# theAdamColton/spiht

Hardware: AMD Instinct MI355X
Metric: Mpixels/sec encode+decode at fixed bpp; bitstream-exact vs Rust ref (higher is better)
Workload: dtype f64 DWT / int32 bit-plane coding; 1 GPU; cfg2 image (1920x1080 RGB, bior2.2 reflect level 7, q=50, 0.5 bpp) x 256 per GPU (cfg4 shard), encode+decode, HBM-resident; images_per_gpu=256, distinct_images_per_gpu=256, seeds=1000 + global image index, streams=1, images_per_launch=256, decoder_waves=8, max_bits=1036800

## Files before the change

### include/spiht_hip.h

```cpp
#ifndef SPIHT_HIP_H
#define SPIHT_HIP_H

#include <stdint.h>

#ifdef __cplusplus
extern "C" {
#endif

enum {
    SPIHT_OK = 0,
    SPIHT_ERR_LL = 1,
    SPIHT_ERR_EMPTY = 2,
    SPIHT_ERR_SHAPE = 3,
    SPIHT_ERR_CAPACITY = 4,
    SPIHT_ERR_HIP = 5,
    SPIHT_ERR_ARG = 6,
    SPIHT_ERR_MAGNITUDE = 7,
    SPIHT_ERR_INTERNAL = 8,
    SPIHT_ERR_TOO_LARGE = 9,
    SPIHT_ERR_NOMEM = 10
};

enum { SPIHT_MODE_REFLECT = 0, SPIHT_MODE_SYMMETRIC = 1, SPIHT_MODE_PERIODIC = 2, SPIHT_MODE_ZERO = 3,
       SPIHT_MODE_CONSTANT = 4,
// ... 423 lines not shown
                          int64_t W, double *d_out);
int spiht_encode_image_batch_flt(spiht_ctx *ctx, int kind, const void *d_img, const int64_t *strides, int64_t B, int64_t c,
                                 int64_t H, int64_t W, int wavelet, int mode, int level, double q_scale,
                                 const double *channel_mults, uint64_t max_bits, uint8_t *d_out, uint64_t slot_stride,
                                 uint64_t *d_nbits, uint8_t *d_max_n, int32_t *d_coeffs);
int spiht_encode_image_host_flt(spiht_ctx *ctx, int kind, const void *img, const int64_t *strides, int64_t c, int64_t H, int64_t W,
                                int wavelet, int mode, int level, double q_scale, const double *channel_mults,
                                uint64_t max_bits, uint8_t *out, uint64_t out_cap, uint64_t *out_nbits, uint8_t *max_n);
int spiht_dwt_pyramid_batch_flt(spiht_ctx *ctx, int kind, const void *d_img, const int64_t *strides, int64_t B, int64_t c, int64_t H,
                                int64_t W, int wavelet, int mode, int level, double q_scale, const double *channel_mults,
                                int32_t *d_coeffs, uint8_t *d_dmsb, uint8_t *d_lmsb, uint32_t *d_maxabs);
int spiht_sse_tiles_flt(spiht_ctx *ctx, int kind, const void *d_tiles, const double *d_dec, int64_t G, int64_t N, int64_t c,
                        int64_t H, int64_t W, int64_t th, int64_t tw, int64_t rh, int64_t rw, double *d_out);
int spiht_sse_tiles_w_flt(spiht_ctx *ctx, int kind, const void *d_tiles, const double *d_dec, int64_t G, int64_t N, int64_t c,
                          int64_t H, int64_t W, int64_t th, int64_t tw, int64_t rh, int64_t rw, double *d_out, const uint8_t *d_w,
                          uint64_t w_stride);
int spiht_tile_cut_f32s(spiht_ctx *ctx, const float *d_img, const int64_t *strides, int64_t N, int64_t c, int64_t H, int64_t W,
                        int64_t th, int64_t tw, float *d_tiles);
int spiht_tile_cut_overlap_f32s(spiht_ctx *ctx, const float *d_img, const int64_t *strides, int64_t N, int64_t c, int64_t H,
                                int64_t W, int64_t th, int64_t tw, int64_t m, float *d_tiles);

int spiht_dwt_addr32(int64_t in_h, int64_t in_w, int64_t out_h, int64_t out_w, int64_t enc_h, int64_t enc_w, int px_es,
                     int64_t px_sh, int64_t px_sw);

enum { SPIHT_ERR_BUSY = 11,
       SPIHT_ERR_TIMEOUT = 12,
       SPIHT_ERR_IDLE = 13 };
enum { SPIHT_HS_ENCODE = 0, SPIHT_HS_DECODE = 1 };
enum { SPIHT_HS_F64 = 0, SPIHT_HS_U8 = 1, SPIHT_HS_U16 = 2,
       SPIHT_HS_FLT32 = 3, SPIHT_HS_FLT16 = 4, SPIHT_HS_BF16 = 5  };
#define SPIHT_HS_DESTROY_MS 10000
typedef struct spiht_hstream spiht_hstream;
typedef struct spiht_hstream_result {
    int64_t n;
    uint64_t nbytes;
    const uint8_t *bytes;
    const uint32_t *lens;
    const uint8_t *max_n;
    void *pictures;
    uint64_t step;
} spiht_hstream_result;
int spiht_hstream_create(spiht_ctx *ctx, int direction, int elem, int64_t B, int depth, int64_t c, int64_t H, int64_t W,
                         int wavelet, int mode, int level, double q_scale, const double *channel_mults, uint64_t max_bits,
                         const int64_t *strides, spiht_hstream **out);
int spiht_hstream_destroy(spiht_hstream *s);
int spiht_hstream_info(spiht_hstream *s, uint64_t *slot_bytes, uint64_t *pic_bytes, int64_t *rec_H, int64_t *rec_W);
// ... 28 lines not shown
```

### spiht_amd/_lib.py

```python
import ctypes as C
import os
import threading

_HERE = os.path.dirname(os.path.abspath(__file__))
LIB_PATH = os.environ.get("SPIHT_HIP_LIB") or os.path.join(_HERE, "libspiht_hip.so")

OK, ERR_LL, ERR_EMPTY, ERR_SHAPE, ERR_CAPACITY, ERR_HIP, ERR_ARG, ERR_MAGNITUDE, ERR_INTERNAL, ERR_TOO_LARGE, \
    ERR_NOMEM = range(11)
ERR_BUSY, ERR_TIMEOUT, ERR_IDLE = 11, 12, 13

MODES = {"reflect": 0, "symmetric": 1, "periodic": 2, "zero": 3, "constant": 4}


class SpihtHipError(RuntimeError):
    """A HIP runtime failure or an internal guard of libspiht_hip."""


class PanicException(BaseException):
    """Counterpart of pyo3_runtime.PanicException, which the reference raises when the Rust core panics
    (assert!(ll_h > 1), encoder_decoder.rs:160-161; out-of-bounds index; unwrap on an empty array).
    Like PyO3's, it derives from BaseException."""


_lib = None
# ... 23 lines not shown
    "spiht_dwt_pyramid_batch_u8", "spiht_dequant_idwt_flags_batch_u8", "spiht_idwt_level1_flags_batch_u8", "spiht_pipeline_submit_u8",
    "spiht_check_view_u8", "spiht_decode_with_metadata_batch_i32",
    "spiht_encode_image_batch_u16", "spiht_decode_image_batch_u16", "spiht_encode_image_host_u16", "spiht_decode_image_host_u16",
    "spiht_dwt_pyramid_batch_u16", "spiht_dequant_idwt_flags_batch_u16", "spiht_idwt_level1_flags_batch_u16", "spiht_pipeline_submit_u16",
    "spiht_check_view_u16",
    "spiht_reduced_shape",
    "spiht_dequant_idwt_reduced_batch_f64", "spiht_dequant_idwt_reduced_batch_u8", "spiht_dequant_idwt_reduced_batch_u16",
    "spiht_decode_image_reduced_batch_f64", "spiht_decode_image_reduced_batch_u8", "spiht_decode_image_reduced_batch_u16",
    "spiht_decode_image_reduced_host_f64", "spiht_decode_image_reduced_host_u8", "spiht_decode_image_reduced_host_u16",
    "spiht_sqerr_i32", "spiht_sse_f64", "spiht_sse_u8", "spiht_sse_u16",
    "spiht_tile_grid", "spiht_tile_cut_u8", "spiht_tile_cut_u16", "spiht_tile_cut_f32", "spiht_tile_cut_f64",
    "spiht_tile_paste_u8", "spiht_tile_paste_u16", "spiht_tile_paste_f32", "spiht_tile_paste_f64",
    "spiht_tile_pack", "spiht_tile_unpack",
    "spiht_tile_reduced_grid", "spiht_tile_mosaic_u8", "spiht_tile_mosaic_u16", "spiht_tile_mosaic_f64",
    "spiht_tile_prefix_slots", "spiht_sse_tiles_f64", "spiht_sse_tiles_u8", "spiht_sse_tiles_u16", "spiht_tile_allocate",
    "spiht_layer_pack", "spiht_layer_unpack",
    "spiht_sse_tiles_w_f64", "spiht_sse_tiles_w_u8", "spiht_sse_tiles_w_u16",
    "spiht_tile_allocate_target",
    "spiht_tile_cut_overlap_u8", "spiht_tile_cut_overlap_u16", "spiht_tile_cut_overlap_f32", "spiht_tile_cut_overlap_f64",
    "spiht_tile_blend_u8", "spiht_tile_blend_u16", "spiht_tile_blend_f64",
    "spiht_check_view_flt", "spiht_convert_batch_flt", "spiht_decode_image_batch_flt", "spiht_decode_image_host_flt",
    "spiht_dequant_idwt_flags_batch_flt", "spiht_dequant_idwt_reduced_batch_flt", "spiht_decode_image_reduced_batch_flt",
    "spiht_decode_image_reduced_host_flt", "spiht_tile_blend_flt", "spiht_tile_paste_f32s", "spiht_tile_mosaic_f32",
    "spiht_dwt_addr32",
    "spiht_widen_batch_flt", "spiht_encode_image_batch_flt", "spiht_encode_image_host_flt", "spiht_dwt_pyramid_batch_flt",
    "spiht_sse_tiles_flt", "spiht_sse_tiles_w_flt", "spiht_tile_cut_f32s", "spiht_tile_cut_overlap_f32s",
    "spiht_hstream_create", "spiht_hstream_destroy", "spiht_hstream_info", "spiht_hstream_input", "spiht_hstream_decode_input",
    "spiht_hstream_submit", "spiht_hstream_next", "spiht_hstream_pending",
    "spiht_tile_cut_set", "spiht_tile_paste_set",
]


class HStreamResult(C.Structure):
    _fields_ = [("n", C.c_int64), ("nbytes", C.c_uint64), ("bytes", C.c_void_p), ("lens", C.c_void_p), ("max_n", C.c_void_p),
                ("pictures", C.c_void_p), ("step", C.c_uint64)]


class TileSetPic(C.Structure):
    _fields_ = [("d_img", C.c_void_p), ("sc", C.c_int64), ("sh", C.c_int64), ("sw", C.c_int64), ("H", C.c_int64), ("W", C.c_int64)]


class TileSetItem(C.Structure):
    _fields_ = [("d_out", C.c_void_p), ("sc", C.c_int64), ("sh", C.c_int64), ("sw", C.c_int64), ("H", C.c_int64), ("W", C.c_int64),
                ("i0", C.c_int64), ("i1", C.c_int64), ("j0", C.c_int64), ("j1", C.c_int64),
                ("y0", C.c_int64), ("x0", C.c_int64), ("wh", C.c_int64), ("ww", C.c_int64)]


# ... 365 lines not shown
```

### spiht_amd/csrc/api_dwt.cpp

```cpp
#include "api_internal.h"
#include "wavelets.h"

static int dwt_max_level(int64_t len, int F) {
    if (F <= 1 || len < F - 1) return 0;
    int64_t q = len / (F - 1);
    int l = 0;
    while (q > 1) { q >>= 1; l++; }
    return l;
}

int img_geometry(int64_t H, int64_t W, int F_real, int level, ImgGeom *g, int mode) {
    if (H < 1 || W < 1) return SPIHT_ERR_ARG;
    int L = level;
    if (L < 0) L = std::min(dwt_max_level(H, F_real), dwt_max_level(W, F_real));
    if (L > SPIHT_MAX_LEVELS) return SPIHT_ERR_ARG;
    g->per = mode == SPIHT_MODE_PERIODIZATION;
    g->l0 = 0;
    const int F = g->per ? 2 : F_real;
    g->L = L;
    g->hs[0] = H;
    g->ws[0] = W;
    for (int l = 1; l <= L; l++) {
        g->hs[l] = (g->hs[l - 1] + F - 1) / 2;
        g->ws[l] = (g->ws[l - 1] + F - 1) / 2;
// ... 380 lines not shown
        CHK(ensure(ctx, ctx->a1, maxa * planes * 8));
    }
    const double *a_in = d_a_in;
    int64_t ah = ig.ll_h, aw = ig.ll_w;
    if (l_hi < ig.L) { ah = 2 * ig.hs[l_hi + 1] - Fg + 2; aw = 2 * ig.ws[l_hi + 1] - Fg + 2; }
    for (int l = l_hi; l >= l_lo; l--) {
        IdwtKArgs a;
        memset(&a, 0, sizeof(a));
        a.c = c;
        a.F = F;
        a.band_h = (int32_t)ig.hs[l]; a.band_w = (int32_t)ig.ws[l];
        a.out_h = (int32_t)(2 * ig.hs[l] - F + 2); a.out_w = (int32_t)(2 * ig.ws[l] - F + 2);
        a.a_h = (int32_t)ah; a.a_w = (int32_t)aw;
        if (!((ah == ig.hs[l] || ah == ig.hs[l] + 1) && (aw == ig.ws[l] || aw == ig.ws[l] + 1))) return SPIHT_ERR_ARG;
        if (ig.per) { a.out_h = (int32_t)(2 * ig.hs[l]); a.out_w = (int32_t)(2 * ig.ws[l]); }
        a.off_h = (int32_t)ig.offh[l]; a.off_w = (int32_t)ig.offw[l];
        a.enc_h = (int32_t)ig.enc_h; a.enc_w = (int32_t)ig.enc_w;
        a.first = (l == ig.L) ? 1 : 0;
        a.a_in = a_in;
        a.rec = d_rec;
        a.out = (l == l_lo) ? d_out : (double *)((l & 1) ? ctx->a1.p : ctx->a0.p);
        a.mults = d_mults;
        a.q = q;
        if (color && l == 1) { a.color = 1; a.col = ctx->col_inv; }
        if (l == 1 && !a.first && !a.color) a.flags = d_flags;
        memcpy(a.lo, wv.rec_lo, sizeof(double) * std::min(F, SPIHT_MAX_TAPS));
        memcpy(a.hi, wv.rec_hi, sizeof(double) * std::min(F, SPIHT_MAX_TAPS));
        const bool conv8 = strided && l == 1 && (ig.per || F > SPIHT_MAX_TAPS);
        if (conv8) {
            CHK(ensure(ctx, ctx->pix, (size_t)planes * a.out_h * a.out_w * 8));
            a.out = (double *)ctx->pix.p;
        }
        if (ig.per || F > SPIHT_MAX_TAPS) {
            const double *d_filt;
            CHK(upload_filters(ctx, wavelet, &d_filt));
            StageTimer t(ctx, l + ig.l0 == 1 ? ST_IDWT_L1 : ST_IDWT_REST);
            a.color = 0;
            const size_t per_plane = (size_t)2 * a.band_h * a.out_w * 8;
            int pc = (int)std::max<size_t>(1, ((size_t)1 << 30) / per_plane);
            pc = std::max(c, pc / c * c);
            CHK(ensure(ctx, ctx->exttmp, per_plane * (size_t)std::min(pc, planes)));
            for (int p0 = 0; p0 < planes; p0 += pc) {
                const int np = std::min(pc, planes - p0);
                IdwtKArgs b = a;
                if (b.a_in) b.a_in = a.a_in + (size_t)p0 * a.a_h * a.a_w;
                b.rec = a.rec + (size_t)p0 * a.enc_h * a.enc_w;
// ... 47 lines not shown
```

### spiht_amd/csrc/common.h

```cpp
#pragma once
#include <hip/hip_runtime.h>
#include <stdint.h>

#define SPIHT_MAX_LEVELS 32
#define SPIHT_MAX_TAPS 20

struct FastDiv {
    uint32_t m, sh, d, pad;
};

static inline FastDiv fastdiv_make(uint32_t d) {
    FastDiv f;
    f.d = d;
    f.pad = 0;
    if (d < 2) { f.m = 0; f.sh = 0; return f; }
    uint32_t l = 0;
    while ((1ull << l) < d) l++;
    uint64_t m = ((1ull << 32) * ((1ull << l) - d)) / d + 1;
    f.m = (uint32_t)m;
    f.sh = l - 1;
    return f;
}

#ifdef __HIPCC__
// ... 233 lines not shown
    int32_t lds_per_cu;
    uint32_t started;
};
#define TILECTR_WORDS (9 * 32)
#define TILECTR_STARTED (8 * 32)
struct TileBase { uint32_t v[8]; };

struct IdwtKArgs {
    int32_t c;
    int32_t F;
    int32_t band_h, band_w;
    int32_t out_h, out_w;
    int32_t a_h, a_w;
    int32_t off_h, off_w, enc_h, enc_w;
    int32_t first;
    int32_t planes;
    const double *a_in;
    const int32_t *rec;
    const uint32_t *flags;
    double *out;
    const double *mults;
    double q;
    double lo[SPIHT_MAX_TAPS], hi[SPIHT_MAX_TAPS];
    int32_t color, pad2;
    Color3 col;
    PxView px;
};

struct LlPicArgs {
    const int32_t *rec;
    int32_t enc_h, enc_w, ll_h, ll_w;
    int32_t c, color;
    const double *mults;
    double q;
    double *out;
    PxView px;
    Color3 col;
};

extern "C" {
int spiht_launch_absmax(const int32_t *d_x, int B, uint32_t n, uint32_t *d_maxabs, hipStream_t st);
int spiht_launch_pyramid(const Geom *g, int B, const int32_t *d_x, uint8_t *d_dmsb, uint8_t *d_lmsb, hipStream_t st);
int spiht_launch_encode(const EncArgs *a, hipStream_t st);
int spiht_launch_encode_wide(const EncArgs *a, const WideArgs *w, int groups, hipStream_t st);
int spiht_wide_groups_per_cu(void);
int spiht_launch_decode(const DecArgs *a, hipStream_t st);
int spiht_launch_decode_w8(const DecArgs *a, hipStream_t st);
int spiht_launch_unscatter(const DecArgs *a, hipStream_t st);
int spiht_meta_sort_temp_bytes(uint64_t rows, size_t *bytes);
int spiht_launch_metadata(const MetaArgs *a, uint32_t *keys_in, uint32_t *vals_in, uint32_t *keys_out, uint32_t *vals_out,
// ... 29 lines not shown
```

### spiht_amd/csrc/dwt_inv.hip

```cpp
#include "dwt_device.h"


template <int F, uint32_t LOM, uint32_t HIM, int PX = PX_F64>
__global__ __launch_bounds__(DW_BLOCK) void k_idwt_level(IdwtKArgs a) {
    constexpr int HF = F / 2;
    constexpr int KH = IW_TH / 2 + HF - 1;
    constexpr int KW = IW_TW / 2 + HF - 1;
    constexpr int KHH = IW_TH / 4 + HF - 1;
    __shared__ double s_b[4][KH][KW + 1];
    uint32_t tbx, tby, tbz;
    xcd_tile((a.out_w + IW_TW - 1) / IW_TW, (a.out_h + IW_TH - 1) / IW_TH, a.planes, tbx, tby, tbz);
    const int plane = (int)tbz;
    const int k = plane % a.c;
    const int m0 = (int)tby * IW_TH, n0 = (int)tbx * IW_TW;
    const int kh0 = m0 / 2, kw0 = n0 / 2;
    const bool has_m = a.mults != nullptr;
    const double mk = has_m ? a.mults[k] : 1.0;
    const bool zero_ok = (!has_m || mk > 0.0) && a.q > 0.0;
    const int32_t *__restrict__ rec = a.rec + (size_t)plane * a.enc_h * a.enc_w;
    const double *__restrict__ ain = a.first ? nullptr : a.a_in + (size_t)plane * a.a_h * a.a_w;
    const int tid = threadIdx.x;
    const bool occupied = a.flags == nullptr ||
        a.flags[((size_t)plane * ((a.out_h + IW_TH - 1) / IW_TH) + tby) * ((a.out_w + IW_TW - 1) / IW_TW) + tbx] != 0u;

// ... 65 lines not shown
                double sa = 0.0, sd = 0.0;
#pragma unroll
                for (int j = 0; j < HF; j++) {
                    const int s = HF - 1 - j;
                    const bool lnz = (LOM >> (mp + F - 2 - 2 * s)) & 1u, hnz = (HIM >> (mp + F - 2 - 2 * s)) & 1u;
                    if (lnz) sa += wl[s] * a.lo[mp + F - 2 - 2 * s];
                    if (hnz) sd += wh[s] * a.hi[mp + F - 2 - 2 * s];
                }
                const double sacc = (0.0 + sa) + sd;
                if (PX) {
                    if (m + mp < a.px.h && n < a.px.w) PX_STORE(PX, out8, (int64_t)(m + mp) * a.px.sh + (int64_t)n * a.px.sw, sacc, a.px.kind);
                } else {
                    if (m + mp < a.out_h && n < a.out_w) out[(size_t)(m + mp) * a.out_w + n] = sacc;
                }
            }
        }
    }
}

#ifndef IWP_WG
#define IWP_WG 4
#endif

template <int F, uint32_t LOM, uint32_t HIM, bool FIRST, bool FLAGS = false, int PX = PX_F64>
__global__ __launch_bounds__(DW_BLOCK) void k_idwt_level_pf(IdwtKArgs a, uint32_t gx, uint32_t gy, uint32_t *ctr,
                                                                      TileBase cb) {
    static_assert(!(FIRST && FLAGS), "the flags are those of level 1 of a transform with two levels or more");
    constexpr int HF = F / 2;
    constexpr int KH = IW_TH / 2 + HF - 1, KW = IW_TW / 2 + HF - 1, KHH = IW_TH / 4 + HF - 1;
    constexpr int NE = (KH * KW + DW_BLOCK - 1) / DW_BLOCK;
    __shared__ double s_b[4][KH][KW + 1];
    const int tid = threadIdx.x;
    const uint32_t nt = gx * gy * (uint32_t)a.planes;
    const uint32_t x = blockIdx.x & 7u, q = nt >> 3, r8 = nt & 7u;
    const uint32_t base = x * q + (x < r8 ? x : r8), cnt = q + (x < r8 ? 1u : 0u);
    __shared__ uint32_t s_next[2];
    uint32_t *const myctr = ctr + 32u * x;
    const uint32_t cbase = cb.v[x];
    if (tid == 0) atomicAdd(ctr + TILECTR_STARTED, 1u);
    uint32_t k, kn;
    if (tid == 0) {
        s_next[0] = atomicAdd(myctr, 1u) - cbase;
        s_next[1] = atomicAdd(myctr, 1u) - cbase;
    }
    __syncthreads();
    k = __builtin_amdgcn_readfirstlane(s_next[0]);
    kn = __builtin_amdgcn_readfirstlane(s_next[1]);
    __syncthreads();

    struct Stage {
        int32_t rad[NE], rda[NE], rdd[NE], raa[NE];
        double vaa[NE];
        double mk;
    };
    auto request = [&](Stage &g, uint32_t T, uint32_t occ) {
        const uint32_t bx = T % gx, t2 = T / gx, by = t2 % gy, plane = t2 / gy;
        const int kh0 = (int)(by * IW_TH) / 2, kw0 = (int)(bx * IW_TW) / 2;
        const int32_t *__restrict__ rec = a.rec + (size_t)plane * a.enc_h * a.enc_w;
        const double *__restrict__ ain = FIRST ? nullptr : a.a_in + (size_t)plane * a.a_h * a.a_w;
        const __amdgpu_buffer_rsrc_t rrsrc = plane_rsrc(rec, (uint32_t)a.enc_h * (uint32_t)a.enc_w * 4u);
#pragma unroll
        for (int e = 0; e < NE; e++) {
            const int p = min(tid + e * DW_BLOCK, KH * KW - 1);
            const int rr = p / KW, cidx = p - rr * KW;
            const int bi = min(kh0 + rr, a.band_h - 1), bj = min(kw0 + cidx, a.band_w - 1);
            if (FLAGS) {
                const uint32_t o_ad = ((uint32_t)bi * (uint32_t)a.enc_w + (uint32_t)(a.off_w + bj)) * 4u;
                const uint32_t o_da = ((uint32_t)(a.off_h + bi) * (uint32_t)a.enc_w + (uint32_t)bj) * 4u;
                g.rad[e] = __builtin_amdgcn_raw_buffer_load_b32(rrsrc, occ ? o_ad : BUF_OOB, 0, 0);
                g.rda[e] = __builtin_amdgcn_raw_buffer_load_b32(rrsrc, occ ? o_da : BUF_OOB, 0, 0);
                g.rdd[e] = __builtin_amdgcn_raw_buffer_load_b32(rrsrc, occ ? o_da + (uint32_t)a.off_w * 4u : BUF_OOB, 0, 0);
            } else {
                g.rad[e] = rec[(size_t)bi * a.enc_w + a.off_w + bj];
                g.rda[e] = rec[(size_t)(a.off_h + bi) * a.enc_w + bj];
                g.rdd[e] = rec[(size_t)(a.off_h + bi) * a.enc_w + a.off_w + bj];
            }
            if (FIRST) { g.raa[e] = rec[(size_t)bi * a.enc_w + bj]; g.vaa[e] = 0.0; }
            else { g.vaa[e] = ain[(size_t)bi * a.a_w + bj]; g.raa[e] = 0; }
        }
        g.mk = a.mults != nullptr ? a.mults[plane % (uint32_t)a.c] : 1.0;
    };
    const int nn = tid & (IW_TW - 1), half = tid / IW_TW, np = nn & 1, cl = nn / 2;
    double tlo[HF], thi[HF];
#pragma unroll
    for (int s2 = 0; s2 < HF; s2++) {
        tlo[s2] = a.lo[np + F - 2 - 2 * s2];
        thi[s2] = a.hi[np + F - 2 - 2 * s2];
    }
    const bool has_m = a.mults != nullptr;
    auto tile = [&](Stage &g, uint32_t kk, uint32_t knext, uint32_t occ_next) {
        const uint32_t T = base + kk;
        const uint32_t bx = T % gx, t2 = T / gx, by = t2 % gy, plane = t2 / gy;
        const int kh0s = (int)(by * IW_TH) / 2, kw0s = (int)(bx * IW_TW) / 2;
        const double mk = g.mk;
        const bool zero_ok = (!has_m || mk > 0.0) && a.q > 0.0;
#pragma unroll
        for (int e = 0; e < NE; e++) {
            const int p = tid + e * DW_BLOCK;
            if (p < KH * KW) {
                const int rr = p / KW, cidx = p - rr * KW;
                const bool in = kh0s + rr < a.band_h && kw0s + cidx < a.band_w;
                const double va = FIRST ? ((g.raa[e] == 0 && zero_ok) ? 0.0 : dequant(g.raa[e], mk, a.q, has_m)) : g.vaa[e];
                s_b[0][rr][cidx] = in ? va : 0.0;
                s_b[1][rr][cidx] = (!in || (g.rad[e] == 0 && zero_ok)) ? 0.0 : dequant(g.rad[e], mk, a.q, has_m);
                s_b[2][rr][cidx] = (!in || (g.rda[e] == 0 && zero_ok)) ? 0.0 : dequant(g.rda[e], mk, a.q, has_m);
                s_b[3][rr][cidx] = (!in || (g.rdd[e] == 0 && zero_ok)) ? 0.0 : dequant(g.rdd[e], mk, a.q, has_m);
            }
        }
        uint32_t drawn = 0;
        if (tid == 0) drawn = atomicAdd(myctr, 1u);
        request(g, base + min(knext, cnt - 1u), occ_next);
        lds_barrier();
        const int m0 = (int)by * IW_TH, n0 = (int)bx * IW_TW, kh0 = m0 / 2;
        const int n = n0 + nn;
        double wl[HF], wh[HF];
#pragma unroll
        for (int s2 = 0; s2 < HF; s2++) { wl[s2] = 0.0; wh[s2] = 0.0; }
        const int rbase = half * (IW_TH / 4);
        const uint32_t row_bytes = (uint32_t)a.out_w * 8u;
        const __amdgpu_buffer_rsrc_t orsrc = PX ? plane_rsrc(a.px.out + (int64_t)(plane / (uint32_t)a.c) * a.px.sb + (int64_t)(plane % (uint32_t)a.c) * a.px.sc,
                                                             (uint32_t)((int64_t)(a.px.h - 1) * a.px.sh + (int64_t)(a.px.w - 1) * a.px.sw + (PX == PX_FLT ? a.px.es : PX)))
                                                : plane_rsrc(a.out + (size_t)plane * a.out_h * a.out_w, (uint32_t)a.out_h * row_bytes);
        const uint32_t voff0 = n < a.out_w ? (uint32_t)(2 * (kh0 + rbase)) * row_bytes + (uint32_t)n * 8u : BUF_OOB;
        const int y0 = 2 * (kh0 + rbase);
        const uint32_t voff8 = n < a.px.w ? (uint32_t)y0 * (uint32_t)a.px.sh + (uint32_t)n * (uint32_t)a.px.sw : BUF_OOB;
#pragma unroll
        for (int rr = 0; rr < KHH; rr++) {
            const int r = rbase + rr;
            double ta = 0.0, td = 0.0, ua = 0.0, ud = 0.0;
#pragma unroll
            for (int j = 0; j < HF; j++) {
                const int s2 = HF - 1 - j;
                constexpr uint32_t PAIR = 3u;
                const bool lnz = ((LOM >> (F - 2 - 2 * s2)) & PAIR) != 0, hnz = ((HIM >> (F - 2 - 2 * s2)) & PAIR) != 0;
                if (lnz) {
                    ta += s_b[0][r][cl + s2] * tlo[s2];
                    ua += s_b[2][r][cl + s2] * tlo[s2];
                }
                if (hnz) {
                    td += s_b[1][r][cl + s2] * thi[s2];
                    ud += s_b[3][r][cl + s2] * thi[s2];
                }
            }
            const double tl = (0.0 + ta) + td, th = (0.0 + ua) + ud;
#pragma unroll
            for (int s2 = 0; s2 < HF - 1; s2++) { wl[s2] = wl[s2 + 1]; wh[s2] = wh[s2 + 1]; }
            wl[HF - 1] = tl;
            wh[HF - 1] = th;
            if (rr >= HF - 1) {
#pragma unroll
                for (int mp = 0; mp < 2; mp++) {
                    double sa = 0.0, sd = 0.0;
#pragma unroll
                    for (int j = 0; j < HF; j++) {
                        const int s2 = HF - 1 - j;
                        const bool lnz = (LOM >> (mp + F - 2 - 2 * s2)) & 1u, hnz = (HIM >> (mp + F - 2 - 2 * s2)) & 1u;
                        if (lnz) sa += wl[s2] * a.lo[mp + F - 2 - 2 * s2];
                        if (hnz) sd += wh[s2] * a.hi[mp + F - 2 - 2 * s2];
                    }
                    const double sacc = (0.0 + sa) + sd;
                    if constexpr (PX == PX_U8) {
                        const int dy = 2 * (rr - (HF - 1)) + mp;
                        __builtin_amdgcn_raw_buffer_store_b8(px8_store_value(sacc), orsrc,
                                                             y0 + dy < a.px.h ? voff8 + (uint32_t)dy * (uint32_t)a.px.sh : BUF_OOB, 0, 0);
                    } else if constexpr (PX == PX_U16) {
                        const int dy = 2 * (rr - (HF - 1)) + mp;
                        __builtin_amdgcn_raw_buffer_store_b16(px16_store_value(sacc), orsrc,
                                                              y0 + dy < a.px.h ? voff8 + (uint32_t)dy * (uint32_t)a.px.sh : BUF_OOB, 0, 0);
                    } else if constexpr (PX == PX_FLT) {
                        const int dy = 2 * (rr - (HF - 1)) + mp;
                        const uint32_t b = flt_store_value(sacc, a.px.kind);
                        const uint32_t vo = y0 + dy < a.px.h ? voff8 + (uint32_t)dy * (uint32_t)a.px.sh : BUF_OOB;
                        __builtin_amdgcn_raw_buffer_store_b32(b, orsrc, a.px.kind == SPIHT_FLT_F32 ? vo : BUF_OOB, 0, 0);
                        __builtin_amdgcn_raw_buffer_store_b16((uint16_t)b, orsrc, a.px.kind == SPIHT_FLT_F32 ? BUF_OOB : vo, 0, 0);
                    } else {
                        __builtin_amdgcn_raw_buffer_store_b64(__builtin_bit_cast(u32x2, sacc), orsrc,
                                                              voff0 + (uint32_t)(2 * (rr - (HF - 1)) + mp) * row_bytes, 0, 0);
                    }
                }
            }
        }
        if (tid == 0) s_next[0] = drawn - cbase;
        lds_barrier();
    };
    Stage g0;
    if (k >= cnt) return;
    auto occupancy = [&](uint32_t kk) -> uint32_t {
        return FLAGS ? a.flags[base + min(kk, cnt - 1u)] : 1u;
    };
    request(g0, base + k, occupancy(k));
    uint32_t occ_n = occupancy(kn);
    tile(g0, k, kn, occ_n);
    k = kn;
    kn = __builtin_amdgcn_readfirstlane(s_next[0]);
    occ_n = occupancy(kn);
    while (k < cnt) {
        tile(g0, k, kn, occ_n);
        k = kn;
        kn = __builtin_amdgcn_readfirstlane(s_next[0]);
        occ_n = occupancy(kn);
    }
}

#define IWC_TH 8
template <int F, uint32_t LOM, uint32_t HIM, int PX = PX_F64>
__global__ __launch_bounds__(DW_BLOCK) void k_idwt1_color(IdwtKArgs a) {
    constexpr int HF = F / 2;
    constexpr int KH = IWC_TH / 2 + HF - 1, KW = IW_TW / 2 + HF - 1, KHH = IWC_TH / 4 + HF - 1;
    __shared__ double s_b[3][4][KH][KW + 1];
    __shared__ SpowLds s_pw;
    spow_lds_fill(s_pw, threadIdx.x);
    uint32_t tbx, tby, tbz;
    xcd_tile((a.out_w + IW_TW - 1) / IW_TW, (a.out_h + IWC_TH - 1) / IWC_TH, a.planes / 3, tbx, tby, tbz);
    const int img = (int)tbz;
    const int m0 = (int)tby * IWC_TH, n0 = (int)tbx * IW_TW;
    const int kh0 = m0 / 2, kw0 = n0 / 2;
    const bool has_m = a.mults != nullptr;
    const int tid = threadIdx.x;
    const size_t cpl = (size_t)a.enc_h * a.enc_w, apl = (size_t)a.a_h * a.a_w, opl = (size_t)a.out_h * a.out_w;

    for (int p = tid; p < 3 * KH * KW; p += DW_BLOCK) {
// ... 82 lines not shown
                    px[ch] = (0.0 + sa) + sd;
                }
                if (PX ? (m + mp < a.px.h && n < a.px.w) : (m + mp < a.out_h && n < a.out_w)) {
                    double w0, w1, w2;
                    color3_px(a.col, s_pw, px[0], px[1], px[2], w0, w1, w2);
                    if (PX) {
                        const int64_t o = (int64_t)(m + mp) * a.px.sh + (int64_t)n * a.px.sw;
                        PX_STORE(PX, out8, o, w0, a.px.kind);
                        PX_STORE(PX, out8, o + a.px.sc, w1, a.px.kind);
                        PX_STORE(PX, out8, o + 2 * a.px.sc, w2, a.px.kind);
                    } else {
                        const size_t o = (size_t)(m + mp) * a.out_w + n;
                        out[o] = w0;
                        out[o + opl] = w1;
                        out[o + 2 * opl] = w2;
                    }
                }
            }
        }
    }
}

template <int F, uint32_t LOM, uint32_t HIM, int PX>
static void launch_idwt_pf(IdwtKArgs &a, uint32_t G, uint32_t pad, hipStream_t st, uint32_t gx, uint32_t gy, uint32_t *ctr, const TileBase &cb) {
    if (a.first) hipLaunchKernelGGL((k_idwt_level_pf<F, LOM, HIM, true, false, PX>), dim3(G), dim3(DW_BLOCK), pad, st, a, gx, gy, ctr, cb);
    else if (a.flags && (uint64_t)a.enc_h * a.enc_w * 4u < (1ull << 31))
        hipLaunchKernelGGL((k_idwt_level_pf<F, LOM, HIM, false, true, PX>), dim3(G), dim3(DW_BLOCK), pad, st, a, gx, gy, ctr, cb);
    else { a.flags = nullptr; hipLaunchKernelGGL((k_idwt_level_pf<F, LOM, HIM, false, false, PX>), dim3(G), dim3(DW_BLOCK), pad, st, a, gx, gy, ctr, cb); }
}
template <int F, uint32_t LOM, uint32_t HIM>
static int launch_idwt_FM(IdwtKArgs a, int planes, hipStream_t st, TileCtr *tc) {
    a.planes = planes;
    const int px = a.px.out == nullptr ? PX_F64 : px_kind_of(a.px);
    if (a.color) {
        uint32_t ntc = (uint32_t)((a.out_w + IW_TW - 1) / IW_TW) * (uint32_t)((a.out_h + IWC_TH - 1) / IWC_TH) * (uint32_t)(planes / 3);
        with_px(px, [&](auto PX) { hipLaunchKernelGGL((k_idwt1_color<F, LOM, HIM, PX>), dim3(ntc), dim3(DW_BLOCK), 0, st, a); });
        return (int)hipGetLastError();
    }
    const uint32_t gx = (uint32_t)((a.out_w + IW_TW - 1) / IW_TW), gy = (uint32_t)((a.out_h + IW_TH - 1) / IW_TH);
    const uint32_t nt = gx * gy * (uint32_t)planes;
    constexpr uint32_t pf_min = 20000u;
    const int num_cu = tc ? tc->num_cu : 0;
    const bool off32 = px ? (uint64_t)((a.px.h - 1) * a.px.sh + (a.px.w - 1) * a.px.sw) + (uint64_t)a.px.es < (1ull << 31)
                          : (uint64_t)(a.out_h + IW_TH) * a.out_w * 8u < (1ull << 31);
    if (tc && tc->dev && num_cu >= 2 && nt >= pf_min && off32) {
        const int g = tc->wg_per_cu > 0 ? tc->wg_per_cu : IWP_WG;
        const uint32_t G = (uint32_t)(num_cu * g);
        uint32_t pad = 0;
        if (g < IWP_WG && tc->lds_per_cu > 0) {
            constexpr int HFk = F / 2;
            constexpr uint32_t own = 4u * (IW_TH / 2 + HFk - 1) * (IW_TW / 2 + HFk) * 8u + 64u;
            const uint32_t want = (uint32_t)tc->lds_per_cu / (uint32_t)(g + 1) + 512u;
            if (want > own && want <= 65536u) pad = want - own;
        }
        TileBase cb;
        uint32_t *ctr = tc->dev;
        for (uint32_t x = 0; x < 8; x++) {
            cb.v[x] = tc->base[x];
            tc->base[x] += (nt >> 3) + (x < (nt & 7u) ? 1u : 0u) + 2u * ((G + 7u - x) >> 3);
        }
        tc->started += G;
        with_px(px, [&](auto PX) { launch_idwt_pf<F, LOM, HIM, PX>(a, G, pad, st, gx, gy, ctr, cb); });
        const hipError_t e = hipGetLastError();
        if (e != hipSuccess) {
            (void)hipMemsetAsync(tc->dev, 0, TILECTR_WORDS * sizeof(uint32_t), st);
            for (uint32_t x = 0; x < 8; x++) tc->base[x] = 0;
            tc->started = 0;
        }
        return (int)e;
    }
    with_px(px, [&](auto PX) { hipLaunchKernelGGL((k_idwt_level<F, LOM, HIM, PX>), dim3(nt), dim3(DW_BLOCK), 0, st, a); });
    return (int)hipGetLastError();
}
template <int F, uint32_t LOM, uint32_t HIM>
static int launch_idwt_F(const IdwtKArgs &a, int planes, hipStream_t st, TileCtr *tc) {
    uint32_t lom, him;
    tap_masks(a.lo, a.hi, F, lom, him);
    if (lom == LOM && him == HIM) return launch_idwt_FM<F, LOM, HIM>(a, planes, st, tc);
    return launch_idwt_FM<F, (1u << F) - 1u, (1u << F) - 1u>(a, planes, st, tc);
}

extern "C" int spiht_launch_idwt_level(const IdwtKArgs *a, int planes, hipStream_t st, TileCtr *tc) {
    switch (a->F) {
    case 2: return launch_idwt_F<2, 0x3u, 0x3u>(*a, planes, st, tc);
    case 6: return launch_idwt_F<6, 0x0Eu, 0x3Eu>(*a, planes, st, tc);
// ... 12 lines not shown
```

Before: 34830 Mpixels/s.

## Streamline persistent IDWT kernel: reciprocal dequant, precomputed address constants, buffer offsets

```diff
diff --git a/include/spiht_hip.h b/include/spiht_hip.h
--- a/include/spiht_hip.h
+++ b/include/spiht_hip.h
@@ -469,6 +469,8 @@
 
 int spiht_dwt_addr32(int64_t in_h, int64_t in_w, int64_t out_h, int64_t out_w, int64_t enc_h, int64_t enc_w, int px_es,
                      int64_t px_sh, int64_t px_sw);
+int spiht_idwt_addr32(int64_t out_h, int64_t out_w, int64_t enc_h, int64_t enc_w, int64_t a_h, int64_t a_w, int first, int px_es,
+                      int64_t px_h, int64_t px_w, int64_t px_sh, int64_t px_sw);
 
 enum { SPIHT_ERR_BUSY = 11,
        SPIHT_ERR_TIMEOUT = 12,
diff --git a/spiht_amd/_lib.py b/spiht_amd/_lib.py
--- a/spiht_amd/_lib.py
+++ b/spiht_amd/_lib.py
@@ -69,7 +69,7 @@
     "spiht_check_view_flt", "spiht_convert_batch_flt", "spiht_decode_image_batch_flt", "spiht_decode_image_host_flt",
     "spiht_dequant_idwt_flags_batch_flt", "spiht_dequant_idwt_reduced_batch_flt", "spiht_decode_image_reduced_batch_flt",
     "spiht_decode_image_reduced_host_flt", "spiht_tile_blend_flt", "spiht_tile_paste_f32s", "spiht_tile_mosaic_f32",
-    "spiht_dwt_addr32",
+    "spiht_dwt_addr32", "spiht_idwt_addr32",
     "spiht_widen_batch_flt", "spiht_encode_image_batch_flt", "spiht_encode_image_host_flt", "spiht_dwt_pyramid_batch_flt",
     "spiht_sse_tiles_flt", "spiht_sse_tiles_w_flt", "spiht_tile_cut_f32s", "spiht_tile_cut_overlap_f32s",
     "spiht_hstream_create", "spiht_hstream_destroy", "spiht_hstream_info", "spiht_hstream_input", "spiht_hstream_decode_input",
diff --git a/spiht_amd/csrc/api_dwt.cpp b/spiht_amd/csrc/api_dwt.cpp
--- a/spiht_amd/csrc/api_dwt.cpp
+++ b/spiht_amd/csrc/api_dwt.cpp
@@ -426,6 +426,8 @@
         a.out = (l == l_lo) ? d_out : (double *)((l & 1) ? ctx->a1.p : ctx->a0.p);
         a.mults = d_mults;
         a.q = q;
+        const bool own_mults = d_mults && d_mults == (const double *)ctx->mults.p && ctx->mults_host.size() == (size_t)c;
+        a.recip_ok = (!d_mults || own_mults) && idwt_recip_ok(q, d_mults ? ctx->mults_host.data() : nullptr, c) ? 1 : 0;
         if (color && l == 1) { a.color = 1; a.col = ctx->col_inv; }
         if (l == 1 && !a.first && !a.color) a.flags = d_flags;
         memcpy(a.lo, wv.rec_lo, sizeof(double) * std::min(F, SPIHT_MAX_TAPS));
diff --git a/spiht_amd/csrc/common.h b/spiht_amd/csrc/common.h
--- a/spiht_amd/csrc/common.h
+++ b/spiht_amd/csrc/common.h
@@ -279,10 +279,47 @@
     const double *mults;
     double q;
     double lo[SPIHT_MAX_TAPS], hi[SPIHT_MAX_TAPS];
-    int32_t color, pad2;
+    int32_t color;
+    int32_t recip_ok;
     Color3 col;
     PxView px;
 };
+
+struct IdwtPfConsts {
+    FastDivU dv_gx, dv_gy, dv_c;
+    uint32_t gx, gy;
+    uint32_t rec_pb, rec_rb;
+    uint32_t so_ad, so_da;
+    uint32_t a_pb, a_rb;
+    uint32_t out_pb, out_rb;
+};
+
+static inline bool idwt_pf_narrow_ok(int64_t out_h, int64_t out_w, int64_t enc_h, int64_t enc_w, int64_t a_h, int64_t a_w, int first,
+                                     int px_es, int64_t px_h, int64_t px_w, int64_t px_sh, int64_t px_sw) {
+    const int64_t lim = (int64_t)1 << 31, row = (int64_t)1 << 24;
+    if (out_h < 1 || out_w < 1 || enc_h < 1 || enc_w < 1) return false;
+    if (out_h >= lim || out_w >= lim || enc_h >= lim || enc_w >= lim) return false;
+    if (px_es) {
+        if (px_h < 1 || px_w < 1 || px_h >= lim || px_w >= lim) return false;
+        if (px_sh < 0 || px_sw < 0 || px_sh >= lim || px_sw >= lim) return false;
+        if ((px_h - 1) * px_sh + (px_w - 1) * px_sw + px_es >= lim) return false;
+    } else if ((out_h + IW_TH) * out_w * 8 >= lim) return false;
+    if (enc_h * enc_w * 4 >= lim || enc_w * 4 >= row) return false;
+    if (!first) {
+        if (a_h < 1 || a_w < 1 || a_h >= lim || a_w >= lim) return false;
+        if (a_h * a_w * 8 >= lim || a_w * 8 >= row) return false;
+    }
+    return true;
+}
+
+static inline bool idwt_recip_ok(double q, const double *mults, int c) {
+    const double lo = 0x1p-500, hi = 0x1p500;
+    if (!(q >= lo && q <= hi)) return false;
+    if (mults)
+        for (int k = 0; k < c; k++)
+            if (!(mults[k] >= lo && mults[k] <= hi && mults[k] * q >= 0x1p-900)) return false;
+    return true;
+}
 
 struct LlPicArgs {
     const int32_t *rec;
diff --git a/spiht_amd/csrc/dwt_inv.hip b/spiht_amd/csrc/dwt_inv.hip
--- a/spiht_amd/csrc/dwt_inv.hip
+++ b/spiht_amd/csrc/dwt_inv.hip
@@ -111,16 +111,39 @@
 #define IWP_WG 4
 #endif
 
+#ifndef IWP_RECIP
+#define IWP_RECIP 1
+#endif
+
+__device__ __forceinline__ double quot_recip(double a, double b, double y) {
+    const double q0 = a * y;
+    const double r0 = __builtin_fma(-b, q0, a);
+    const double q1 = __builtin_fma(r0, y, q0);
+    const double r1 = __builtin_fma(-b, q1, a);
+    return __builtin_fma(r1, y, q1);
+}
+__device__ __forceinline__ double dequant_recip(int32_t r, double m, double ym, double q, double yq, bool has_m) {
+    double v = (double)r;
+#if IWP_RECIP
+    if (has_m) v = quot_recip(v, m, ym);
+    return quot_recip(v, q, yq);
+#else
+    if (has_m) v = v / m;
+    return v / q;
+#endif
+}
+
+#define IWP_REGS96(F, LOM) ((F) <= 4 || ((F) == 6 && (LOM) == 0x0Eu))
 template <int F, uint32_t LOM, uint32_t HIM, bool FIRST, bool FLAGS = false, int PX = PX_F64>
-__global__ __launch_bounds__(DW_BLOCK) void k_idwt_level_pf(IdwtKArgs a, uint32_t gx, uint32_t gy, uint32_t *ctr,
-                                                                      TileBase cb) {
+__global__ __launch_bounds__(DW_BLOCK, IWP_REGS96(F, LOM) ? 5 : 1) void k_idwt_level_pf(IdwtKArgs a, IdwtPfConsts kc, uint32_t *ctr, TileBase cb) {
+    constexpr bool REGS96 = IWP_REGS96(F, LOM);
     static_assert(!(FIRST && FLAGS), "the flags are those of level 1 of a transform with two levels or more");
     constexpr int HF = F / 2;
     constexpr int KH = IW_TH / 2 + HF - 1, KW = IW_TW / 2 + HF - 1, KHH = IW_TH / 4 + HF - 1;
     constexpr int NE = (KH * KW + DW_BLOCK - 1) / DW_BLOCK;
     __shared__ double s_b[4][KH][KW + 1];
     const int tid = threadIdx.x;
-    const uint32_t nt = gx * gy * (uint32_t)a.planes;
+    const uint32_t nt = kc.gx * kc.gy * (uint32_t)a.planes;
     const uint32_t x = blockIdx.x & 7u, q = nt >> 3, r8 = nt & 7u;
     const uint32_t base = x * q + (x < r8 ? x : r8), cnt = q + (x < r8 ? 1u : 0u);
     __shared__ uint32_t s_next[2];
@@ -142,32 +165,65 @@
         double vaa[NE];
         double mk;
     };
-    auto request = [&](Stage &g, uint32_t T, uint32_t occ) {
-        const uint32_t bx = T % gx, t2 = T / gx, by = t2 % gy, plane = t2 / gy;
-        const int kh0 = (int)(by * IW_TH) / 2, kw0 = (int)(bx * IW_TW) / 2;
-        const int32_t *__restrict__ rec = a.rec + (size_t)plane * a.enc_h * a.enc_w;
-        const double *__restrict__ ain = FIRST ? nullptr : a.a_in + (size_t)plane * a.a_h * a.a_w;
-        const __amdgpu_buffer_rsrc_t rrsrc = plane_rsrc(rec, (uint32_t)a.enc_h * (uint32_t)a.enc_w * 4u);
+    struct Tile {
+        uint32_t kh0, kw0;
+        uint32_t plane;
+    };
+    auto tile_at = [&](uint32_t T) -> Tile {
+        const uint32_t t2 = fdivu(T, kc.dv_gx), bx = T - t2 * kc.gx;
+        const uint32_t plane = fdivu(t2, kc.dv_gy), by = t2 - plane * kc.gy;
+        return Tile{by * (uint32_t)(IW_TH / 2), bx * (uint32_t)(IW_TW / 2), plane};
+    };
+    uint32_t e_r[NE], e_c4[NE];
+    auto elem_at = [&](int t, int e, uint32_t &r, uint32_t &c4) {
+        const int p = min(t + e * DW_BLOCK, KH * KW - 1);
+        const int rr = p / KW;
+        r = (uint32_t)rr;
+        c4 = (uint32_t)(p - rr * KW) * 4u;
+    };
+#pragma unroll
+    for (int e = 0; e < NE; e++) elem_at(tid, e, e_r[e], e_c4[e]);
+    auto elem = [&](int e, uint32_t &r, uint32_t &c4) {
+        if constexpr (REGS96) {
+            r = e_r[e];
+            c4 = e_c4[e];
+        } else {
+            int t = tid;
+            asm volatile("" : "+v"(t));
+            elem_at(t, e, r, c4);
+        }
+    };
+    auto request = [&](Stage &g, const Tile &t, uint32_t occ) {
+        const __amdgpu_buffer_rsrc_t rrsrc = plane_rsrc((const char *)a.rec + (uint64_t)t.plane * kc.rec_pb, FLAGS && !occ ? 0u : kc.rec_pb);
+        const uint32_t lim_r = (uint32_t)a.band_h - 1u - t.kh0, lim_c4 = ((uint32_t)a.band_w - 1u - t.kw0) * 4u;
+        const uint32_t so_aa = t.kh0 * kc.rec_rb + t.kw0 * 4u;
+        const uint32_t so_ad = so_aa + kc.so_ad, so_da = so_aa + kc.so_da, so_dd = so_da + kc.so_ad;
+        __amdgpu_buffer_rsrc_t arsrc = rrsrc;
+        uint32_t so_a = 0;
+        if (!FIRST) {
+            arsrc = plane_rsrc((const char *)a.a_in + (uint64_t)t.plane * kc.a_pb, kc.a_pb);
+            so_a = t.kh0 * kc.a_rb + t.kw0 * 8u;
+        }
 #pragma unroll
         for (int e = 0; e < NE; e++) {
-            const int p = min(tid + e * DW_BLOCK, KH * KW - 1);
-            const int rr = p / KW, cidx = p - rr * KW;
-            const int bi = min(kh0 + rr, a.band_h - 1), bj = min(kw0 + cidx, a.band_w - 1);
-            if (FLAGS) {
-                const uint32_t o_ad = ((uint32_t)bi * (uint32_t)a.enc_w + (uint32_t)(a.off_w + bj)) * 4u;
-                const uint32_t o_da = ((uint32_t)(a.off_h + bi) * (uint32_t)a.enc_w + (uint32_t)bj) * 4u;
-                g.rad[e] = __builtin_amdgcn_raw_buffer_load_b32(rrsrc, occ ? o_ad : BUF_OOB, 0, 0);
-                g.rda[e] = __builtin_amdgcn_raw_buffer_load_b32(rrsrc, occ ? o_da : BUF_OOB, 0, 0);
-                g.rdd[e] = __builtin_amdgcn_raw_buffer_load_b32(rrsrc, occ ? o_da + (uint32_t)a.off_w * 4u : BUF_OOB, 0, 0);
+            uint32_t er, ec4;
+            elem(e, er, ec4);
+            const uint32_t rm = min(er, lim_r), cm = min(ec4, lim_c4);
+            const uint32_t vo = __umul24(rm, kc.rec_rb) + cm;
+            g.rad[e] = __builtin_amdgcn_raw_buffer_load_b32(rrsrc, vo, so_ad, 0);
+            g.rda[e] = __builtin_amdgcn_raw_buffer_load_b32(rrsrc, vo, so_da, 0);
+            g.rdd[e] = __builtin_amdgcn_raw_buffer_load_b32(rrsrc, vo, so_dd, 0);
+            if (FIRST) {
+                g.raa[e] = __builtin_amdgcn_raw_buffer_load_b32(rrsrc, vo, so_aa, 0);
+                g.vaa[e] = 0.0;
             } else {
-                g.rad[e] = rec[(size_t)bi * a.enc_w + a.off_w + bj];
-                g.rda[e] = rec[(size_t)(a.off_h + bi) * a.enc_w + bj];
-                g.rdd[e] = rec[(size_t)(a.off_h + bi) * a.enc_w + a.off_w + bj];
-            }
-            if (FIRST) { g.raa[e] = rec[(size_t)bi * a.enc_w + bj]; g.vaa[e] = 0.0; }
-            else { g.vaa[e] = ain[(size_t)bi * a.a_w + bj]; g.raa[e] = 0; }
-        }
-        g.mk = a.mults != nullptr ? a.mults[plane % (uint32_t)a.c] : 1.0;
+                g.vaa[e] = __builtin_bit_cast(double, __builtin_amdgcn_raw_buffer_load_b64(arsrc, __umul24(rm, kc.a_rb) + 2u * cm, so_a, 0));
+                g.raa[e] = 0;
+            }
+        }
+        double mk = 1.0;
+        if (a.mults != nullptr) mk = a.mults[t.plane - fdivu(t.plane, kc.dv_c) * (uint32_t)a.c];
+        g.mk = mk;
     };
     const int nn = tid & (IW_TW - 1), half = tid / IW_TW, np = nn & 1, cl = nn / 2;
     double tlo[HF], thi[HF];
@@ -177,40 +233,57 @@
         thi[s2] = a.hi[np + F - 2 - 2 * s2];
     }
     const bool has_m = a.mults != nullptr;
-    auto tile = [&](Stage &g, uint32_t kk, uint32_t knext, uint32_t occ_next) {
-        const uint32_t T = base + kk;
-        const uint32_t bx = T % gx, t2 = T / gx, by = t2 % gy, plane = t2 / gy;
-        const int kh0s = (int)(by * IW_TH) / 2, kw0s = (int)(bx * IW_TW) / 2;
+    const uint32_t st_rel = (uint32_t)(2 * (half * (IW_TH / 4))) * kc.out_rb + (uint32_t)nn * 8u;
+    const double yq = 1.0 / a.q;
+    auto tile = [&](Stage &g, const Tile &t, const Tile &tnext, uint32_t occ_next) {
+        const uint32_t plane = t.plane;
+        const uint32_t lim_r = (uint32_t)a.band_h - 1u - t.kh0, lim_c4 = ((uint32_t)a.band_w - 1u - t.kw0) * 4u;
         const double mk = g.mk;
+        const double ym = has_m && IWP_RECIP ? 1.0 / mk : 1.0;
         const bool zero_ok = (!has_m || mk > 0.0) && a.q > 0.0;
 #pragma unroll
         for (int e = 0; e < NE; e++) {
-            const int p = tid + e * DW_BLOCK;
-            if (p < KH * KW) {
-                const int rr = p / KW, cidx = p - rr * KW;
-                const bool in = kh0s + rr < a.band_h && kw0s + cidx < a.band_w;
-                const double va = FIRST ? ((g.raa[e] == 0 && zero_ok) ? 0.0 : dequant(g.raa[e], mk, a.q, has_m)) : g.vaa[e];
-                s_b[0][rr][cidx] = in ? va : 0.0;
-                s_b[1][rr][cidx] = (!in || (g.rad[e] == 0 && zero_ok)) ? 0.0 : dequant(g.rad[e], mk, a.q, has_m);
-                s_b[2][rr][cidx] = (!in || (g.rda[e] == 0 && zero_ok)) ? 0.0 : dequant(g.rda[e], mk, a.q, has_m);
-                s_b[3][rr][cidx] = (!in || (g.rdd[e] == 0 && zero_ok)) ? 0.0 : dequant(g.rdd[e], mk, a.q, has_m);
+            if (tid + e * DW_BLOCK < KH * KW) {
+                uint32_t er, ec4;
+                elem(e, er, ec4);
+                const bool in = er <= lim_r && ec4 <= lim_c4;
+                double *const cell = reinterpret_cast<double *>(reinterpret_cast<char *>(&s_b[0][0][0]) + er * (uint32_t)((KW + 1) * 8) + ec4 * 2u);
+                constexpr int BAND = KH * (KW + 1);
+                double vaa = FIRST ? 0.0 : (in ? g.vaa[e] : 0.0), vad = 0.0, vda = 0.0, vdd = 0.0;
+                if (in && (!zero_ok || (g.rad[e] | g.rda[e] | g.rdd[e] | (FIRST ? g.raa[e] : 0)) != 0)) {
+                    if (FIRST) vaa = dequant_recip(g.raa[e], mk, ym, a.q, yq, has_m);
+                    vad = dequant_recip(g.rad[e], mk, ym, a.q, yq, has_m);
+                    vda = dequant_recip(g.rda[e], mk, ym, a.q, yq, has_m);
+                    vdd = dequant_recip(g.rdd[e], mk, ym, a.q, yq, has_m);
+                }
+                cell[0] = vaa;
+                cell[BAND] = vad;
+                cell[2 * BAND] = vda;
+                cell[3 * BAND] = vdd;
             }
         }
         uint32_t drawn = 0;
         if (tid == 0) drawn = atomicAdd(myctr, 1u);
-        request(g, base + min(knext, cnt - 1u), occ_next);
+        request(g, tnext, occ_next);
         lds_barrier();
-        const int m0 = (int)by * IW_TH, n0 = (int)bx * IW_TW, kh0 = m0 / 2;
+        const int n0 = (int)(2u * t.kw0), kh0 = (int)t.kh0;
         const int n = n0 + nn;
         double wl[HF], wh[HF];
 #pragma unroll
         for (int s2 = 0; s2 < HF; s2++) { wl[s2] = 0.0; wh[s2] = 0.0; }
         const int rbase = half * (IW_TH / 4);
-        const uint32_t row_bytes = (uint32_t)a.out_w * 8u;
-        const __amdgpu_buffer_rsrc_t orsrc = PX ? plane_rsrc(a.px.out + (int64_t)(plane / (uint32_t)a.c) * a.px.sb + (int64_t)(plane % (uint32_t)a.c) * a.px.sc,
-                                                             (uint32_t)((int64_t)(a.px.h - 1) * a.px.sh + (int64_t)(a.px.w - 1) * a.px.sw + (PX == PX_FLT ? a.px.es : PX)))
-                                                : plane_rsrc(a.out + (size_t)plane * a.out_h * a.out_w, (uint32_t)a.out_h * row_bytes);
-        const uint32_t voff0 = n < a.out_w ? (uint32_t)(2 * (kh0 + rbase)) * row_bytes + (uint32_t)n * 8u : BUF_OOB;
+        int clt = cl;
+        if constexpr (!REGS96) asm volatile("" : "+v"(clt));
+        const uint32_t row_bytes = kc.out_rb;
+        __amdgpu_buffer_rsrc_t orsrc;
+        if constexpr (PX != PX_F64) {
+            const uint32_t img = fdivu(plane, kc.dv_c), ch = plane - img * (uint32_t)a.c;
+            orsrc = plane_rsrc(a.px.out + (int64_t)img * a.px.sb + (int64_t)ch * a.px.sc,
+                               (uint32_t)((int64_t)(a.px.h - 1) * a.px.sh + (int64_t)(a.px.w - 1) * a.px.sw + (PX == PX_FLT ? a.px.es : PX)));
+        } else {
+            orsrc = plane_rsrc((char *)a.out + (uint64_t)plane * kc.out_pb, kc.out_pb);
+        }
+        uint32_t vst = n < a.out_w ? st_rel + (2u * t.kh0 * row_bytes + (uint32_t)n0 * 8u) : BUF_OOB;
         const int y0 = 2 * (kh0 + rbase);
         const uint32_t voff8 = n < a.px.w ? (uint32_t)y0 * (uint32_t)a.px.sh + (uint32_t)n * (uint32_t)a.px.sw : BUF_OOB;
 #pragma unroll
@@ -223,12 +296,12 @@
                 constexpr uint32_t PAIR = 3u;
                 const bool lnz = ((LOM >> (F - 2 - 2 * s2)) & PAIR) != 0, hnz = ((HIM >> (F - 2 - 2 * s2)) & PAIR) != 0;
                 if (lnz) {
-                    ta += s_b[0][r][cl + s2] * tlo[s2];
-                    ua += s_b[2][r][cl + s2] * tlo[s2];
+                    ta += s_b[0][r][clt + s2] * tlo[s2];
+                    ua += s_b[2][r][clt + s2] * tlo[s2];
                 }
                 if (hnz) {
-                    td += s_b[1][r][cl + s2] * thi[s2];
-                    ud += s_b[3][r][cl + s2] * thi[s2];
+                    td += s_b[1][r][clt + s2] * thi[s2];
+                    ud += s_b[3][r][clt + s2] * thi[s2];
                 }
             }
             const double tl = (0.0 + ta) + td, th = (0.0 + ua) + ud;
@@ -263,8 +336,8 @@
                         __builtin_amdgcn_raw_buffer_store_b32(b, orsrc, a.px.kind == SPIHT_FLT_F32 ? vo : BUF_OOB, 0, 0);
                         __builtin_amdgcn_raw_buffer_store_b16((uint16_t)b, orsrc, a.px.kind == SPIHT_FLT_F32 ? BUF_OOB : vo, 0, 0);
                     } else {
-                        __builtin_amdgcn_raw_buffer_store_b64(__builtin_bit_cast(u32x2, sacc), orsrc,
-                                                              voff0 + (uint32_t)(2 * (rr - (HF - 1)) + mp) * row_bytes, 0, 0);
+                        __builtin_amdgcn_raw_buffer_store_b64(__builtin_bit_cast(u32x2, sacc), orsrc, vst, 0, 0);
+                        vst += row_bytes;
                     }
                 }
             }
@@ -277,15 +350,19 @@
     auto occupancy = [&](uint32_t kk) -> uint32_t {
         return FLAGS ? a.flags[base + min(kk, cnt - 1u)] : 1u;
     };
-    request(g0, base + k, occupancy(k));
+    Tile tc = tile_at(base + k), tn = tile_at(base + min(kn, cnt - 1u));
+    request(g0, tc, occupancy(k));
     uint32_t occ_n = occupancy(kn);
-    tile(g0, k, kn, occ_n);
+    tile(g0, tc, tn, occ_n);
     k = kn;
+    tc = tn;
     kn = __builtin_amdgcn_readfirstlane(s_next[0]);
     occ_n = occupancy(kn);
     while (k < cnt) {
-        tile(g0, k, kn, occ_n);
+        tn = tile_at(base + min(kn, cnt - 1u));
+        tile(g0, tc, tn, occ_n);
         k = kn;
+        tc = tn;
         kn = __builtin_amdgcn_readfirstlane(s_next[0]);
         occ_n = occupancy(kn);
     }
@@ -414,11 +491,31 @@
 }
 
 template <int F, uint32_t LOM, uint32_t HIM, int PX>
-static void launch_idwt_pf(IdwtKArgs &a, uint32_t G, uint32_t pad, hipStream_t st, uint32_t gx, uint32_t gy, uint32_t *ctr, const TileBase &cb) {
-    if (a.first) hipLaunchKernelGGL((k_idwt_level_pf<F, LOM, HIM, true, false, PX>), dim3(G), dim3(DW_BLOCK), pad, st, a, gx, gy, ctr, cb);
-    else if (a.flags && (uint64_t)a.enc_h * a.enc_w * 4u < (1ull << 31))
-        hipLaunchKernelGGL((k_idwt_level_pf<F, LOM, HIM, false, true, PX>), dim3(G), dim3(DW_BLOCK), pad, st, a, gx, gy, ctr, cb);
-    else { a.flags = nullptr; hipLaunchKernelGGL((k_idwt_level_pf<F, LOM, HIM, false, false, PX>), dim3(G), dim3(DW_BLOCK), pad, st, a, gx, gy, ctr, cb); }
+static void launch_idwt_pf(IdwtKArgs &a, const IdwtPfConsts &kc, uint32_t G, uint32_t pad, hipStream_t st, uint32_t *ctr, const TileBase &cb) {
+    if (a.first) hipLaunchKernelGGL((k_idwt_level_pf<F, LOM, HIM, true, false, PX>), dim3(G), dim3(DW_BLOCK), pad, st, a, kc, ctr, cb);
+    else if (a.flags) hipLaunchKernelGGL((k_idwt_level_pf<F, LOM, HIM, false, true, PX>), dim3(G), dim3(DW_BLOCK), pad, st, a, kc, ctr, cb);
+    else hipLaunchKernelGGL((k_idwt_level_pf<F, LOM, HIM, false, false, PX>), dim3(G), dim3(DW_BLOCK), pad, st, a, kc, ctr, cb);
+}
+extern "C" int spiht_idwt_addr32(int64_t out_h, int64_t out_w, int64_t enc_h, int64_t enc_w, int64_t a_h, int64_t a_w, int first,
+                                 int px_es, int64_t px_h, int64_t px_w, int64_t px_sh, int64_t px_sw) {
+    return idwt_pf_narrow_ok(out_h, out_w, enc_h, enc_w, a_h, a_w, first, px_es, px_h, px_w, px_sh, px_sw) ? 1 : 0;
+}
+static IdwtPfConsts idwt_set_launch_consts(const IdwtKArgs &a, uint32_t gx, uint32_t gy) {
+    IdwtPfConsts kc;
+    kc.gx = gx;
+    kc.gy = gy;
+    kc.dv_gx = fastdivu_make(gx);
+    kc.dv_gy = fastdivu_make(gy);
+    kc.dv_c = fastdivu_make((uint32_t)a.c);
+    kc.rec_pb = (uint32_t)a.enc_h * (uint32_t)a.enc_w * 4u;
+    kc.rec_rb = (uint32_t)a.enc_w * 4u;
+    kc.so_ad = (uint32_t)a.off_w * 4u;
+    kc.so_da = (uint32_t)a.off_h * kc.rec_rb;
+    kc.a_pb = a.first ? 0u : (uint32_t)a.a_h * (uint32_t)a.a_w * 8u;
+    kc.a_rb = a.first ? 0u : (uint32_t)a.a_w * 8u;
+    kc.out_pb = (uint32_t)a.out_h * (uint32_t)a.out_w * 8u;
+    kc.out_rb = (uint32_t)a.out_w * 8u;
+    return kc;
 }
 template <int F, uint32_t LOM, uint32_t HIM>
 static int launch_idwt_FM(IdwtKArgs a, int planes, hipStream_t st, TileCtr *tc) {
@@ -433,9 +530,10 @@
     const uint32_t nt = gx * gy * (uint32_t)planes;
     constexpr uint32_t pf_min = 20000u;
     const int num_cu = tc ? tc->num_cu : 0;
-    const bool off32 = px ? (uint64_t)((a.px.h - 1) * a.px.sh + (a.px.w - 1) * a.px.sw) + (uint64_t)a.px.es < (1ull << 31)
-                          : (uint64_t)(a.out_h + IW_TH) * a.out_w * 8u < (1ull << 31);
-    if (tc && tc->dev && num_cu >= 2 && nt >= pf_min && off32) {
+    const bool off32 = spiht_idwt_addr32(a.out_h, a.out_w, a.enc_h, a.enc_w, a.a_h, a.a_w, a.first, px ? a.px.es : 0, a.px.h, a.px.w,
+                                         a.px.sh, a.px.sw) != 0;
+    const bool quot_ok = !IWP_RECIP || a.recip_ok;
+    if (tc && tc->dev && num_cu >= 2 && nt >= pf_min && off32 && quot_ok) {
         const int g = tc->wg_per_cu > 0 ? tc->wg_per_cu : IWP_WG;
         const uint32_t G = (uint32_t)(num_cu * g);
         uint32_t pad = 0;
@@ -452,7 +550,8 @@
             tc->base[x] += (nt >> 3) + (x < (nt & 7u) ? 1u : 0u) + 2u * ((G + 7u - x) >> 3);
         }
         tc->started += G;
-        with_px(px, [&](auto PX) { launch_idwt_pf<F, LOM, HIM, PX>(a, G, pad, st, gx, gy, ctr, cb); });
+        const IdwtPfConsts kc = idwt_set_launch_consts(a, gx, gy);
+        with_px(px, [&](auto PX) { launch_idwt_pf<F, LOM, HIM, PX>(a, kc, G, pad, st, ctr, cb); });
         const hipError_t e = hipGetLastError();
         if (e != hipSuccess) {
             (void)hipMemsetAsync(tc->dev, 0, TILECTR_WORDS * sizeof(uint32_t), st);
```

Result: no change. 35020 Mpixels/s (median of 2 runs) (+0.5%).
